# Zhang-Xin-Duke/multimodal-detection-consistency

Hardware: AMD Instinct MI355X
Metric: defended queries/sec (higher is better)
Workload: dtype bf16; 1 GPU; ViT-L/14 bf16, batch=512/GPU, N=8 variants, 1000000-row bf16 bank, encode + exact top-5 bank search + consistency (BASELINE configs[2]); global_batch=512, parallelism=dp1, text_packing=eot-packed + variant prefix sharing (bit-identical, see DESIGN.md), bank=gaussian + planted neighbours of the text rows

## Files before the change

multimodal-detection-consistency_amd/csrc/elementwise.hip:

```cpp
#include "common.hpp"
#include "kernels.hpp"
#include "launch.hpp"
#include "rows.hpp"

#ifndef TVC_LN_NT
#define TVC_LN_NT 7
#endif

template <bool F16>
__global__ __launch_bounds__(256) void layernorm_kernel(float* __restrict__ x, int64_t x_row_stride,
                                                        const int32_t* __restrict__ row_idx,
                                                        const uint16_t* __restrict__ delta,
                                                        const uint16_t* __restrict__ delta2, int write_x,
                                                        const float* __restrict__ g,
                                                        const float* __restrict__ b,
                                                        uint16_t* __restrict__ y, int rows, int d,
                                                        int delta_compact, float* __restrict__ xsum_out,
                                                        float* __restrict__ y32) {
    const int lane = row_lane();
    const int row = wave_row();
    if (row >= rows) return;
    const int64_t src_row = row_idx ? (int64_t)row_idx[row] : (int64_t)row;
    f32x4_t* xr = (f32x4_t*)(x + src_row * x_row_stride);
    const int64_t doff = delta_compact ? (int64_t)row * d : src_row * x_row_stride;
    const u32x2_t* dr = delta ? (const u32x2_t*)(delta + doff) : nullptr;
    const u32x2_t* dr2 = delta2 ? (const u32x2_t*)(delta2 + doff) : nullptr;
    const int nv = d >> 2;
    f32x4_t v[4] = {};
    float s = 0.f;
    for_pieces(lane, nv, [&](int i, int c) {
#if TVC_LN_NT & 1
        v[i] = __builtin_nontemporal_load(xr + c);
#else
        v[i] = xr[c];
#endif
        if (dr) {
#if TVC_LN_NT & 4
            v[i] += unpack4<F16>(__builtin_nontemporal_load(dr + c));
#else
            v[i] += unpack4<F16>(dr[c]);
#endif
        }
        if (dr2) v[i] += unpack4<F16>(dr2[c]);
#if TVC_LN_NT & 2
        if (write_x && (dr || dr2)) __builtin_nontemporal_store(v[i], xr + c);
#else
        if (write_x && (dr || dr2)) xr[c] = v[i];
#endif
        if (xsum_out) ((f32x4_t*)(xsum_out + (int64_t)row * d))[c] = v[i];
        s += piece_sum(v[i]);
    });
    const float mean = row_mean(s, d);
    const float rstd = row_rstd(v, mean, lane, nv, d);
    u32x2_t* yr = (u32x2_t*)(y + (int64_t)row * d);
    for_pieces(lane, nv, [&](int i, int c) {
        const f32x4_t o = ln_affine(v[i], mean, rstd, g, b, c);
        if (y32) ((f32x4_t*)(y32 + (int64_t)row * d))[c] = o;
        if (y) {
#if TVC_LN_NT & 8
            __builtin_nontemporal_store(pack4<F16>(o), yr + c);
#else
            yr[c] = pack4<F16>(o);
#endif
        }
    });
}

hipError_t launch_layernorm(float* x, int64_t x_row_stride, const int32_t* row_idx, const uint16_t* delta,
                            int write_x, const float* g, const float* b, uint16_t* y, int rows, int d,
                            hipStream_t stream, const uint16_t* delta2, int delta_compact, float* xsum_out, float* y32,
                            int f16) {
    if (d % 4 != 0 || d > 1024 || rows < 0) return hipErrorInvalidValue;
    if (rows == 0) return hipSuccess;
    return dispatch<true, false>(f16 != 0, [&](auto h) {
        return launch<layernorm_kernel<h.value>>(row_grid(rows), dim3(256), 0, stream, x, x_row_stride, row_idx, delta, delta2, write_x, g, b,
                                                 y, rows, d, delta_compact, xsum_out, y32);
    });
}

template <bool F16>
__global__ __launch_bounds__(256) void im2col_kernel(const float* __restrict__ pix,
                                                     uint16_t* __restrict__ out, int B, int S,
                                                     int patch, int Kp) {
    const int g = S / patch;
    const int P = g * g;
    const int chunks = Kp >> 3;
    const int64_t total = (int64_t)B * P * chunks;
    const int K = 3 * patch * patch;
    for (int64_t t = (int64_t)blockIdx.x * blockDim.x + threadIdx.x; t < total;
         t += (int64_t)gridDim.x * blockDim.x) {
        const int ch = (int)(t % chunks);
        const int64_t row = t / chunks;
        const int p = (int)(row % P);
        const int bimg = (int)(row / P);
        const int py = p / g, px = p - py * g;
        uint32_t w[4];
#pragma unroll
        for (int e = 0; e < 4; ++e) {
            float f[2];
#pragma unroll
            for (int h = 0; h < 2; ++h) {
                const int col = ch * 8 + e * 2 + h;
                float val = 0.f;
                if (col < K) {
                    const int c = col / (patch * patch);
                    const int rem = col - c * patch * patch;
                    const int ky = rem / patch, kx = rem - ky * patch;
                    val = pix[(((int64_t)bimg * 3 + c) * S + (py * patch + ky)) * S + (px * patch + kx)];
                }
                f[h] = val;
            }
            w[e] = Op16<F16>::pack2(f[0], f[1]);
        }
        *(u32x4_t*)(out + row * Kp + ch * 8) = u32x4_t{w[0], w[1], w[2], w[3]};
    }
}

template <bool F16>
__global__ __launch_bounds__(256) void im2col_rows_kernel(const float* __restrict__ pix, uint16_t* __restrict__ out,
                                                          int S, int patch, int Kp) {
    extern __shared__ __attribute__((aligned(16))) char im_smem[];
    uint16_t* tile = (uint16_t*)im_smem;
    const int g = S / patch;
    const int bimg = blockIdx.x / g, py = blockIdx.x - bimg * g;
    const int K = 3 * patch * patch;
    for (int i = threadIdx.x; i < g * (Kp - K); i += 256) {
        const int px = i / (Kp - K), c = K + (i - px * (Kp - K));
        tile[px * Kp + c] = 0;
    }
    const int s4 = S >> 2;
    const int total = 3 * patch * s4;
    for (int i = threadIdx.x; i < total; i += 256) {
        const int rowi = i / s4, x4 = i - rowi * s4;
        const int c = rowi / patch, ky = rowi - c * patch;
        const f32x4_t v = __builtin_nontemporal_load(
            (const f32x4_t*)(pix + (((int64_t)bimg * 3 + c) * S + (py * patch + ky)) * S) + x4);
#pragma unroll
        for (int e = 0; e < 4; ++e) {
            const int x = x4 * 4 + e;
            const int px = x / patch, kx = x - px * patch;
            tile[px * Kp + c * patch * patch + ky * patch + kx] = Op16<F16>::from_f32(v[e]);
        }
    }
    __syncthreads();
    const int chunks = (g * Kp) >> 3;
    u32x4_t* dst = (u32x4_t*)(out + ((int64_t)bimg * g * g + (int64_t)py * g) * Kp);
    for (int i = threadIdx.x; i < chunks; i += 256) dst[i] = ((const u32x4_t*)tile)[i];
}

hipError_t launch_im2col(const float* pix, uint16_t* out, int B, int image, int patch, int Kp,
                         hipStream_t stream, int f16) {
    if (B <= 0) return hipSuccess;
    const int g = image / patch;
    const size_t lds = (size_t)g * Kp * 2;
    if (image % 4 == 0 && Kp % 8 == 0 && lds <= 64 * 1024)
        return dispatch<true, false>(f16 != 0, [&](auto h) {
            return launch<im2col_rows_kernel<h.value>>(dim3(B * g), dim3(256), lds, stream, pix, out, image, patch, Kp);
        });
    const int64_t total = (int64_t)B * g * g * (Kp >> 3);
    return dispatch<true, false>(f16 != 0, [&](auto h) {
        return launch<im2col_kernel<h.value>>(stride_grid(total, 8192), dim3(256), 0, stream, pix, out, B, image, patch, Kp);
    });
}

__global__ __launch_bounds__(256) void assemble_lnpre_kernel(const float* __restrict__ patch_out,
                                                             const float* __restrict__ cls,
                                                             const float* __restrict__ pos,
                                                             const float* __restrict__ g,
                                                             const float* __restrict__ b,
                                                             float* __restrict__ x, int B, int T, int d) {
    const int lane = row_lane();
    const int64_t row = wave_row<int64_t>();
    if (row >= (int64_t)B * T) return;
    const int t = (int)(row % T);
    const int64_t bimg = row / T;
    const f32x4_t* src = (t == 0) ? (const f32x4_t*)cls
                                  : (const f32x4_t*)(patch_out + (bimg * (T - 1) + (t - 1)) * d);
    const f32x4_t* pr = (const f32x4_t*)(pos + (int64_t)t * d);
    const int nv = d >> 2;
    f32x4_t v[4] = {};
    float s = 0.f;
    for_pieces(lane, nv, [&](int i, int c) {
        v[i] = src[c] + pr[c];
        s += piece_sum(v[i]);
    });
    const float mean = row_mean(s, d);
    const float rstd = row_rstd(v, mean, lane, nv, d);
    f32x4_t* xr = (f32x4_t*)(x + row * d);
    for_pieces(lane, nv, [&](int i, int c) { xr[c] = ln_affine(v[i], mean, rstd, g, b, c); });
}

hipError_t launch_assemble_lnpre(const float* patch_out, const float* cls, const float* pos,
                                 const float* g, const float* b, float* x, int B, int T, int d,
                                 hipStream_t stream) {
    if (d % 4 != 0 || d > 1024) return hipErrorInvalidValue;
    const int64_t rows = (int64_t)B * T;
    if (rows == 0) return hipSuccess;
    return launch<assemble_lnpre_kernel>(row_grid(rows), dim3(256), 0, stream, patch_out, cls, pos, g, b, x, B, T, d);
}

__device__ __forceinline__ int first_max_pos(const int32_t* __restrict__ tok, int ctx, int lane) {
    int best = -1, best_t = 0;
    for (int tt = lane; tt < ctx; tt += 64) {
        const int v = tok[tt];
        if (v > best) { best = v; best_t = tt; }
    }
#pragma unroll
    for (int o = 32; o > 0; o >>= 1) {
        const int ov = __shfl_xor(best, o, 64);
        const int ot = __shfl_xor(best_t, o, 64);
        if (ov > best || (ov == best && ot < best_t)) { best = ov; best_t = ot; }
    }
    return best_t;
}

__global__ __launch_bounds__(256) void text_lens_kernel(const int32_t* __restrict__ tok, int32_t* __restrict__ starts,
                                                        int32_t* __restrict__ pfx, int32_t* __restrict__ lens,
                                                        int n_text, int ctx, int G) {
    const int lane = row_lane();
    const int n = wave_row();
    if (n >= n_text) return;
    int len = first_max_pos(tok + (int64_t)n * ctx, ctx, lane) + 1, p = 0;
    if (pfx) {
        const int bn = n / G * G;
        if (bn != n) {
            int bb = -1, bt = 0, mis = 0x7fffffff;
            for (int tt = lane; tt < ctx; tt += 64) {
                const int vb = tok[(int64_t)bn * ctx + tt], vn = tok[(int64_t)n * ctx + tt];
                if (vb > bb) { bb = vb; bt = tt; }
                if (vb != vn && tt < mis) mis = tt;
            }
#pragma unroll
            for (int o = 32; o > 0; o >>= 1) {
                const int ov = __shfl_xor(bb, o, 64);
                const int ot = __shfl_xor(bt, o, 64);
                if (ov > bb || (ov == bb && ot < bt)) { bb = ov; bt = ot; }
                const int om = __shfl_xor(mis, o, 64);
                mis = om < mis ? om : mis;
            }
            p = mis;
            if (p > len) p = len;
            if (p > bt + 1) p = bt + 1;
        }
        if (lane == 0) pfx[n] = p;
    }
    if (lane == 0) { starts[n] = len - p; lens[n] = len; }
}

__global__ __launch_bounds__(1024) void text_scan_kernel(int32_t* __restrict__ starts, int32_t* __restrict__ pfx,
                                                         const int32_t* __restrict__ lens, int n_text, int G) {
    __shared__ int part[1024];
// ... 192 lines not shown
```

multimodal-detection-consistency_amd/csrc/kernels.hpp:

```cpp
#pragma once
#include <hip/hip_runtime.h>
#include <stdint.h>
#include "host_plan.hpp"

enum { TVC_EPI_F32 = 0, TVC_EPI_BF16 = 1, TVC_EPI_GELU_BF16 = 2, TVC_EPI_RESID_F32 = 3 };

struct GemmLaunch {
    const uint16_t* A = nullptr;
    const uint16_t* B = nullptr;
    int64_t lda = 0, ldb = 0;
    int I = 0, J = 0, K = 0;
    int planes = 1;
    int a_plane_off[9] = {0, 0, 0, 0, 0, 0, 0, 0, 0};
    int b_plane_off[9] = {0, 0, 0, 0, 0, 0, 0, 0, 0};
    bool splitk_small = false;
    int splitk_fixed = 0;
    bool a_rows_padded = false;
    const float* bias = nullptr;
    void* out = nullptr;
    int64_t ldo = 0;
    int epilogue = TVC_EPI_F32;
    bool b_rows_padded = false;
    float* splitk_ws = nullptr;
    size_t splitk_ws_bytes = 0;
    bool f16 = false;
};
hipError_t launch_gemm_bf16(const GemmLaunch& L, hipStream_t stream);
inline GemmLaunch gemm_launch(const uint16_t* A, int64_t lda, int I, const uint16_t* B, int64_t ldb, int J, int K,
                              const float* bias, void* out, int64_t ldo, int epilogue) {
    GemmLaunch g;
    g.A = A; g.lda = lda; g.I = I; g.B = B; g.ldb = ldb; g.J = J; g.K = K;
    g.bias = bias; g.out = out; g.ldo = ldo; g.epilogue = epilogue;
    return g;
}
inline GemmLaunch gemm_launch_planes(const uint16_t* A, int64_t lda, int I, int bank_planes, const uint16_t* B, int J, int D,
                                     float* out, int64_t ldo) {
    GemmLaunch g = gemm_launch(A, lda, I, B, 2 * (int64_t)D, J, D, nullptr, out, ldo, TVC_EPI_F32);
    g.planes = bank_planes == 2 ? 3 : 2;
    g.b_plane_off[1] = D;
    g.a_plane_off[2] = D;
    return g;
}
inline GemmFormArgs form_args(const GemmLaunch& L) {
    GemmFormArgs a;
    a.I = L.I; a.J = L.J; a.K = L.K; a.planes = L.planes; a.lda = L.lda; a.ldb = L.ldb; a.epilogue = L.epilogue;
    a.splitk_small = L.splitk_small; a.splitk_fixed = L.splitk_fixed; a.has_ws = L.splitk_ws != nullptr;
    a.ws_bytes = L.splitk_ws_bytes; a.a_rows_padded = L.a_rows_padded; a.b_rows_padded = L.b_rows_padded;
    return a;
}

hipError_t launch_layernorm(float* x, int64_t x_row_stride, const int32_t* row_idx, const uint16_t* delta,
                            int write_x, const float* g, const float* b, uint16_t* y, int rows, int d,
                            hipStream_t stream, const uint16_t* delta2 = nullptr, int delta_compact = 0,
                            float* xsum_out = nullptr,
                            float* y32 = nullptr,
                            int f16 = 0);
hipError_t launch_im2col(const float* pix, uint16_t* out, int B, int image, int patch, int Kp,
                         hipStream_t stream, int f16 = 0);
hipError_t launch_assemble_lnpre(const float* patch_out, const float* cls, const float* pos,
                                 const float* g, const float* b, float* x, int B, int T, int d,
                                 hipStream_t stream);
hipError_t launch_text_embed(const int32_t* tok, const float* tok_emb, const float* pos, float* x,
                             int32_t* eot_row, const int32_t* starts, int n_text, int ctx, int d, int vocab,
                             hipStream_t stream, const int32_t* pfx = nullptr);
hipError_t launch_text_lens_scan(const int32_t* tok, int32_t* starts, int32_t* pfx, int n_text, int ctx, int G,
                                 hipStream_t stream, int32_t* lens_ws);
hipError_t launch_l2norm_rows(float* x, int rows, int d, hipStream_t stream);
hipError_t launch_gelu_erf_16(uint16_t* x, int64_t n, int f16, hipStream_t stream);
hipError_t launch_gelu_erf_f32(float* x, int64_t n, hipStream_t stream);
hipError_t launch_split_planes(const float* x, uint16_t* out, int64_t rows, int d, int planes,
                               hipStream_t stream);
hipError_t launch_gather_rows(const uint16_t* bank, int64_t ld, int planes, int D, int64_t R,
                              const int32_t* idx, int64_t idx_offset, int n, float* out,
                              hipStream_t stream);

hipError_t launch_attention(const uint16_t* qkv, uint16_t* out, const int32_t* starts, int n_seq,
                            int seq_len, int heads, int causal, hipStream_t stream, const int32_t* pfx = nullptr,
                            int pool_mode = 0, const int32_t* pool_row = nullptr,
                            int f16 = 0);

struct BankSearchLaunch {
    const uint16_t* bank = nullptr;
    int64_t ldb = 0;
    int64_t R = 0;
    int D = 0;
    int bank_planes = 1;
    const uint16_t* qplanes = nullptr;
    const float* rows = nullptr;
    const float* bank_bounds = nullptr;
    bool allow_filter = true;
    bool q_rows_padded = false;
    int M = 0;
    int k = 0;
    float count_thr = 0.f;
    int64_t idx_offset = 0;
    float* s0 = nullptr;
    float* gmax = nullptr;
    float* tau = nullptr;
    void* cand = nullptr;
    int32_t* cand_cnt = nullptr;
    float* mom_part = nullptr;
    int32_t* overflow = nullptr;
    int n_sample = 0, sample_stride = 1, S = 0, cap = 0;
    int32_t* topk_idx = nullptr;
    float* topk_sim = nullptr;
    float* moments = nullptr;
};
hipError_t launch_bank_search(const BankSearchLaunch& L, hipStream_t stream);
hipError_t launch_bank_bounds(const uint16_t* bank, int64_t ld, int planes, int D, int64_t R, float* bounds,
                              hipStream_t stream);
hipError_t launch_bank_search_dense(const BankSearchLaunch& L, float* sims_ws, int block_rows, hipStream_t stream);
hipError_t launch_topk_merge(const int32_t* idx_parts, const float* sim_parts, const float* feat_parts,
                             const float* mom_parts, int W, int M, int k, int kf, int D,
                             int32_t* idx_out, float* sim_out, float* feat_out, float* mom_out,
                             hipStream_t stream);

struct ConsistencyParams {
    int reference_count;
    float similarity_threshold;
    int retrieval_top_k;
    float dup_threshold;
    float w_text_variants, w_consistency;
    float w_exp[4];
};
// ... 63 lines not shown
```

multimodal-detection-consistency_amd/csrc/rows.hpp:

```cpp
#pragma once
#include "common.hpp"

#define ROWS_PER_BLOCK 4
#define LN_EPS 1e-5f

__device__ __forceinline__ int row_lane() { return threadIdx.x & 63; }
template <class R = int>
__device__ __forceinline__ R wave_row() { return (R)blockIdx.x * ROWS_PER_BLOCK + (threadIdx.x >> 6); }

template <class F>
__device__ __forceinline__ void for_pieces(int lane, int nv, F&& f) {
#pragma unroll
    for (int i = 0; i < 4; ++i) {
        const int c = lane + 64 * i;
        if (c < nv) f(i, c);
    }
}

__device__ __forceinline__ float piece_sum(const f32x4_t v) { return (v[0] + v[1]) + (v[2] + v[3]); }
__device__ __forceinline__ float row_mean(float s, int d) { return wave_sum(s) / (float)d; }
template <bool EXACT = false>
__device__ __forceinline__ float row_rstd(const f32x4_t (&v)[4], float mean, int lane, int nv, int d) {
    float q = 0.f;
    for_pieces(lane, nv, [&](int i, int) {
#pragma unroll
        for (int t = 0; t < 4; ++t) {
#pragma clang fp contract(off)
            const float dl = v[i][t] - mean;
            q += dl * dl;
        }
    });
    const float var = wave_sum(q) / (float)d + LN_EPS;
    return EXACT ? 1.0f / sqrtf(var) : rsqrtf(var);
}

__device__ __forceinline__ f32x4_t ln_affine(const f32x4_t v, float mean, float rstd, const float* __restrict__ g,
                                             const float* __restrict__ b, int c) {
    const f32x4_t gg = ((const f32x4_t*)g)[c];
    const f32x4_t bb = ((const f32x4_t*)b)[c];
    f32x4_t o;
#pragma unroll
    for (int t = 0; t < 4; ++t) o[t] = fmaf((v[t] - mean) * rstd, gg[t], bb[t]);
    return o;
}

template <class Store>
__device__ __forceinline__ void ln_bwd_tail(f32x4_t (&v)[4], const f32x4_t (&g)[4], float mean, float rstd, int lane, int nv,
                                            int d, Store&& store) {
    float sg = 0.f, sgx = 0.f;
    for_pieces(lane, nv, [&](int i, int) {
#pragma unroll
        for (int t = 0; t < 4; ++t) {
            v[i][t] = (v[i][t] - mean) * rstd;
            sg += g[i][t];
            sgx = fmaf(g[i][t], v[i][t], sgx);
        }
    });
    const float c1 = wave_sum(sg) / (float)d, c2 = wave_sum(sgx) / (float)d;
    for_pieces(lane, nv, [&](int i, int c) {
        f32x4_t o;
#pragma unroll
        for (int t = 0; t < 4; ++t) o[t] = rstd * (g[i][t] - c1 - v[i][t] * c2);
        store(c, o);
    });
}

__device__ __forceinline__ float gelu_erf(float x) { return 0.5f * x * (1.0f + erff(x * 0.70710678118654752f)); }
__device__ __forceinline__ float quick_gelu_sigmoid(float x) {
    return __builtin_amdgcn_rcpf(1.0f + __builtin_amdgcn_exp2f(-2.4554670f * x));
}
__device__ __forceinline__ float quick_gelu(float x) { return x * quick_gelu_sigmoid(x); }
__device__ __forceinline__ float quick_gelu_grad(float x) {
    const float s = quick_gelu_sigmoid(x);
    return s + 1.702f * x * s * (1.0f - s);
}
__device__ __forceinline__ float quick_gelu_exact(float x) { return x / (1.0f + expf(-1.702f * x)); }

template <bool F16 = false>
__device__ __forceinline__ f32x4_t unpack4(const u32x2_t w) {
    return f32x4_t{Op16<F16>::lo(w[0]), Op16<F16>::hi(w[0]), Op16<F16>::lo(w[1]), Op16<F16>::hi(w[1])};
}
template <bool F16 = false>
__device__ __forceinline__ u32x2_t pack4(const f32x4_t f) {
    return u32x2_t{Op16<F16>::pack2(f[0], f[1]), Op16<F16>::pack2(f[2], f[3])};
}
template <bool F16 = false>
__device__ __forceinline__ void unpack8(const u32x4_t v, float* f) {
#pragma unroll
    for (int i = 0; i < 4; ++i) {
        f[2 * i] = Op16<F16>::lo(v[i]);
        f[2 * i + 1] = Op16<F16>::hi(v[i]);
    }
}
template <bool F16 = false>
__device__ __forceinline__ u32x4_t pack8(const float* f) {
    return u32x4_t{Op16<F16>::pack2(f[0], f[1]), Op16<F16>::pack2(f[2], f[3]), Op16<F16>::pack2(f[4], f[5]),
// ... 3 lines not shown
```

multimodal-detection-consistency_amd/csrc/tvc_abi.cpp:

```cpp
#include "handle.hpp"

#include <cstdlib>

namespace {

bool tower_ok(const tvc_tower_arch& a) {
    return a.width > 0 && a.layers > 0 && a.heads > 0 && a.width == a.heads * 64 && a.width % 64 == 0 &&
           a.width <= 1024 && a.mlp > 0 && a.mlp % 64 == 0 && (a.act == TVC_ACT_QUICK_GELU || a.act == TVC_ACT_GELU);
}

struct PoolBufs { uint16_t *Hc, *D1c, *H2c, *MLPc, *D2c; };
PoolBufs pool_bufs(tvc_handle* h, const tvc_tower_arch& a, int n_seq, int wso) {
    uint16_t* p = (uint16_t*)h->ws[WS_POOL + wso].p;
    const size_t nd = ((size_t)n_seq + 256) * a.width;
    PoolBufs b;
    b.Hc = p; b.D1c = p + nd; b.H2c = p + 2 * nd; b.D2c = p + 3 * nd; b.MLPc = p + 4 * nd;
    return b;
}
size_t pool_bytes(const tvc_tower_arch& a, int n_seq) {
    return (((size_t)n_seq + 256) * a.width * 4 + ((size_t)n_seq + 256) * a.mlp) * 2;
}

struct GradSave {
    float* x;
    uint16_t* qkv;
    uint16_t* d1;
    uint16_t* u;
};

int run_layers(tvc_handle* h, const tvc_tower_arch& a, const tvc_layer_weights* lw, int n_seq, int seq_len,
               int causal, const int32_t* starts, int total_rows, int wso, hipStream_t st,
               const int32_t* pfx = nullptr, int pool_mode = 0, const int32_t* pool_row = nullptr,
               int64_t pool_x_stride = 0, const GradSave* gs = nullptr, bool f16 = false) {
    const int d = a.width;
    const int rows = starts ? total_rows : n_seq * seq_len;
    float* X = (float*)h->ws[WS_X + wso].p;
    uint16_t* H = (uint16_t*)h->ws[WS_H + wso].p;
    uint16_t* QKV = (uint16_t*)h->ws[WS_QKV + wso].p;
    uint16_t* MLP = (uint16_t*)h->ws[WS_MLP + wso].p;
    uint16_t* D1 = (uint16_t*)h->ws[WS_DELTA + wso].p;
    uint16_t* D2 = (uint16_t*)h->ws[WS_DELTA2 + wso].p;
    bool pending = false;
    for (int l = 0; l < a.layers; ++l) {
        const tvc_layer_weights& w = lw[l];
        {
            ProfScope ps(h, st, TVC_PROF_ROWOPS, (double)rows * d * (pending ? 14.0 : 6.0));
            HIP_TRY(launch_layernorm(X, d, nullptr, pending ? D1 : nullptr, 1, w.ln1_g, w.ln1_b, H, rows, d, st,
                                     pending ? D2 : nullptr, 0, gs ? gs->x + (size_t)l * rows * d : nullptr, nullptr, f16));
        }
        if (gs) {
            QKV = gs->qkv + (size_t)l * rows * 3 * d;
            D1 = gs->d1 + (size_t)l * rows * d;
        }
        GemmLaunch g = gemm_launch(w.wqkv, d, 3 * d, H, d, rows, d, w.bqkv, QKV, 3 * d, TVC_EPI_BF16);
        g.b_rows_padded = true; g.f16 = f16;
        g.splitk_small = gs != nullptr;
        HIP_TRY(timed_gemm(h, g, st, WS_SPLITK + wso));
        if (pool_mode && l == a.layers - 1) {
            const PoolBufs pb = pool_bufs(h, a, n_seq, wso);
            {
                const double avg_len = starts ? (double)rows / n_seq : (double)seq_len;
                ProfScope ps(h, st, TVC_PROF_ATTENTION, 4.0 * n_seq * a.heads * avg_len * 64);
                HIP_TRY(launch_attention(QKV, pb.Hc, starts, n_seq, seq_len, a.heads, causal, st, pfx, pool_mode, pool_row, f16));
            }
            g = gemm_launch(w.wo, d, d, pb.Hc, d, n_seq, d, w.bo, pb.D1c, d, TVC_EPI_BF16);
            g.b_rows_padded = true; g.f16 = f16;
            HIP_TRY(timed_gemm(h, g, st, WS_SPLITK + wso));
            HIP_TRY(launch_layernorm(X, pool_row ? d : pool_x_stride, pool_row, pb.D1c, 0, w.ln2_g, w.ln2_b, pb.H2c, n_seq, d,
                                     st, nullptr, 1, nullptr, nullptr, f16));
            g = gemm_launch(w.w1, d, a.mlp, pb.H2c, d, n_seq, d, w.b1, pb.MLPc, a.mlp,
                            a.act == TVC_ACT_GELU ? TVC_EPI_BF16 : TVC_EPI_GELU_BF16);
            g.b_rows_padded = true; g.f16 = f16;
            HIP_TRY(timed_gemm(h, g, st, WS_SPLITK + wso));
            if (a.act == TVC_ACT_GELU)
                HIP_TRY(launch_gelu_erf_16(pb.MLPc, (int64_t)n_seq * a.mlp, f16, st));
            g = gemm_launch(w.w2, a.mlp, d, pb.MLPc, a.mlp, n_seq, a.mlp, w.b2, pb.D2c, d, TVC_EPI_BF16);
            g.b_rows_padded = true; g.f16 = f16;
            HIP_TRY(timed_gemm(h, g, st, WS_SPLITK + wso));
            return TVC_OK;
        }
        {
            const double avg_len = starts ? (double)rows / n_seq : (double)seq_len;
            const double fl = 4.0 * n_seq * a.heads * avg_len * avg_len * 64 * (causal ? 0.5 : 1.0);
            ProfScope ps(h, st, TVC_PROF_ATTENTION, fl);
            HIP_TRY(launch_attention(QKV, H, starts, n_seq, seq_len, a.heads, causal, st, pfx, 0, nullptr, f16));
        }
        g = gemm_launch(w.wo, d, d, H, d, rows, d, w.bo, D1, d, TVC_EPI_BF16);
        g.b_rows_padded = true; g.f16 = f16; g.splitk_small = gs != nullptr;
        HIP_TRY(timed_gemm(h, g, st, WS_SPLITK + wso));
        {
            ProfScope ps(h, st, TVC_PROF_ROWOPS, (double)rows * d * 8.0);
            HIP_TRY(launch_layernorm(X, d, nullptr, D1, 0, w.ln2_g, w.ln2_b, H, rows, d, st, nullptr, 0, nullptr, nullptr, f16));
        }
        uint16_t* U = gs ? gs->u + (size_t)l * rows * a.mlp : MLP;
        g = gemm_launch(w.w1, d, a.mlp, H, d, rows, d, w.b1, U, a.mlp, gs || a.act == TVC_ACT_GELU ? TVC_EPI_BF16 : TVC_EPI_GELU_BF16);
        g.b_rows_padded = true; g.f16 = f16; g.splitk_small = gs != nullptr;
        HIP_TRY(timed_gemm(h, g, st, WS_SPLITK + wso));
        if (gs) {
            HIP_TRY(launch_gelu_fwd(U, MLP, (int64_t)rows * a.mlp, st));
        } else if (a.act == TVC_ACT_GELU) {
            ProfScope ps(h, st, TVC_PROF_ROWOPS, (double)rows * a.mlp * 4.0);
            HIP_TRY(launch_gelu_erf_16(MLP, (int64_t)rows * a.mlp, f16, st));
        }
        g = gemm_launch(w.w2, a.mlp, d, MLP, a.mlp, rows, a.mlp, w.b2, D2, d, TVC_EPI_BF16);
        g.b_rows_padded = true; g.f16 = f16; g.splitk_small = gs != nullptr;
        HIP_TRY(timed_gemm(h, g, st, WS_SPLITK + wso));
        pending = true;
    }
    return TVC_OK;
}

int ensure_tower_ws(tvc_handle* h, const tvc_tower_arch& a, int64_t rows, int n_seq, int wso) {
// ... 6 lines not shown
    if ((rc = ensure(h, (Slot)(WS_CLS + wso), (size_t)n_seq * a.width * 2))) return rc;
    if ((rc = ensure(h, (Slot)(WS_DELTA + wso), (size_t)rows * a.width * 2))) return rc;
    if ((rc = ensure(h, (Slot)(WS_DELTA2 + wso), (size_t)rows * a.width * 2))) return rc;
    if ((rc = ensure(h, (Slot)(WS_SPLITK + wso), (size_t)256 * 256 * 256 * 4))) return rc;
    if ((rc = ensure(h, (Slot)(WS_POOL + wso), pool_bytes(a, n_seq)))) return rc;
    return TVC_OK;
}

int patch_stem(tvc_handle* h, const char* fn, const float* pix, int n, bool f16, const float** patch_out, hipStream_t st) {
    const tvc_model_desc& m = h->desc;
    const int gside = m.image_size / m.patch, P = gside * gside, d = m.vision.width;
    const int Kp = (3 * m.patch * m.patch + 63) / 64 * 64;
    uint16_t* Pm = (uint16_t*)h->ws[WS_PATCH].p;
    float* po = (float*)h->ws[WS_MLP].p;
    if ((size_t)n * P * d * 4 > h->ws[WS_MLP].n) return fail(h, TVC_E_INVALID, std::string(fn) + ": mlp < 2*width unsupported");
    HIP_TRY(launch_im2col(pix, Pm, n, m.image_size, m.patch, Kp, st, f16));
    GemmLaunch g = gemm_launch((f16 ? h->vision16 : h->vision).w.patch_w, Kp, d, Pm, Kp, n * P, Kp, nullptr, po, d, TVC_EPI_F32);
    g.b_rows_padded = true; g.f16 = f16;
    HIP_TRY(timed_gemm(h, g, st, WS_SPLITK));
    *patch_out = po;
    return TVC_OK;
}


int tower_begin(tvc_handle* h, bool text, const char* fn, int n_seq, float** X) {
    const int mode = h->tower_precision;
    auto missing = [&](const char* tail) {
        return fail(h, TVC_E_STATE, std::string(mode == 3 ? fn : text ? "tvc_encode_text" : "tvc_encode_image") +
                                        ": TVC_OPT_TOWER_PRECISION = " + std::to_string(mode) + " needs tvc_set_weights_f" +
                                        (mode == 3 ? "16" : "32") + (text ? " (text)" : " (vision)") + tail);
    };
    const bool has32 = text ? h->text32.set : h->vision32.set;
    if (mode == 1) return has32 ? precise_ensure(h, text, n_seq, X) : missing("");
    if (mode == 2) {
        if (!has32 || !h->split_ready || (text ? h->tsplit : h->vsplit).empty()) return missing(" before the option is set");
        return split_ensure(h, text, n_seq, X);
    }
    if (mode == 3 && !(text ? h->text16.set : h->vision16.set)) return missing("");
    const tvc_model_desc& m = h->desc;
    const int gside = m.image_size / m.patch, P = gside * gside, T = P + 1;
    const int Kp = (3 * m.patch * m.patch + 63) / 64 * 64;
    int rc;
    if (text) {
        if ((rc = ensure_tower_ws(h, m.text, (int64_t)n_seq * m.ctx, n_seq, WS_TOWER_N))) return rc;
    } else {
        if ((rc = ensure_tower_ws(h, m.vision, (int64_t)n_seq * T, n_seq, 0))) return rc;
        if ((rc = ensure(h, WS_PATCH, ((size_t)n_seq * P + 512) * Kp * 2))) return rc;
    }
    *X = (float*)h->ws[WS_X + (text ? WS_TOWER_N : 0)].p;
    return TVC_OK;
}

int tower_layers(tvc_handle* h, bool text, int n_seq, int seq_len, const int32_t* starts, int total_rows, const int32_t* pfx,
                 bool pool, int64_t x_stride, const int32_t* row_idx, hipStream_t st) {
    if (h->tower_precision == 1) return precise_layers(h, text, n_seq, seq_len, st);
    if (h->tower_precision == 2) return split_layers(h, text, n_seq, seq_len, starts, total_rows, pfx, st);
    const bool f16 = h->tower_precision == 3;
    const tvc_layer_weights* lw = text ? (f16 ? h->text16 : h->text).w.layers : (f16 ? h->vision16 : h->vision).w.layers;
    return run_layers(h, text ? h->desc.text : h->desc.vision, lw, n_seq, seq_len, text ? 1 : 0, starts, total_rows,
                      text ? WS_TOWER_N : 0, st, pfx, pool ? (text ? 2 : 1) : 0, row_idx, x_stride, nullptr, f16);
}

int tower_head(tvc_handle* h, bool text, int64_t x_stride, const int32_t* row_idx, int rows, bool pool, float* out, bool hidden,
               hipStream_t st) {
    if (h->tower_precision == 1) return precise_head(h, text, x_stride, row_idx, rows, out, hidden, st);
    if (h->tower_precision == 2) return split_head(h, text, x_stride, row_idx, rows, out, hidden, st);
    const bool f16 = h->tower_precision == 3;
    const tvc_model_desc& m = h->desc;
    const tvc_tower_arch& a = text ? m.text : m.vision;
    const int d = a.width, wso = text ? WS_TOWER_N : 0;
    const tvc_vision_weights& vw = (f16 ? h->vision16 : h->vision).w;
    const tvc_text_weights& tw = (f16 ? h->text16 : h->text).w;
    const PoolBufs pb = pool ? pool_bufs(h, a, rows, wso) : PoolBufs{};
    uint16_t* Hc = hidden ? nullptr : (uint16_t*)h->ws[WS_CLS + wso].p;
    HIP_TRY(launch_layernorm((float*)h->ws[WS_X + wso].p, x_stride, row_idx, pool ? pb.D1c : (const uint16_t*)h->ws[WS_DELTA + wso].p,
                             0, text ? tw.ln_final_g : vw.ln_post_g, text ? tw.ln_final_b : vw.ln_post_b, Hc, rows, d, st,
                             pool ? pb.D2c : (const uint16_t*)h->ws[WS_DELTA2 + wso].p, pool ? 1 : 0, nullptr,
                             hidden ? out : nullptr, f16));
    if (hidden) return TVC_OK;
    GemmLaunch g = gemm_launch(text ? tw.proj : vw.proj, d, m.embed_dim, Hc, d, rows, d, nullptr, out, m.embed_dim, TVC_EPI_F32);
    g.f16 = f16;
    HIP_TRY(timed_gemm(h, g, st, WS_SPLITK + wso));
    return TVC_OK;
}

int encode_text(tvc_handle* h, const char* fn, const int32_t* tok_dev, int32_t Tn, float* out_dev, int32_t normalize, bool hidden,
                void* stream) {
    if (!h) return TVC_E_INVALID;
    if (!h->text.set) return fail(h, TVC_E_STATE, std::string(fn) + ": handle has no text tower");
    if (Tn < 0 || (Tn > 0 && (!tok_dev || !out_dev))) return fail(h, TVC_E_INVALID, std::string(fn) + ": bad arguments");
    hipStream_t st = (hipStream_t)stream;
    const tvc_model_desc& m = h->desc;
    const int d = m.text.width, ctx = m.ctx;
    if (Tn == 0) return TVC_OK;
    int chunk = Tn < h->max_chunk_texts ? Tn : h->max_chunk_texts;
    const int mode = h->tower_precision;
    const bool pack = h->pack_text && !hidden && mode != 1;
    const bool pool = h->pooled_last && !hidden && (mode == 0 || mode == 3);
    const int G = (pack && h->text_group >= 2 && Tn % h->text_group == 0) ? h->text_group : 0;
    if (G && chunk >= G) chunk = chunk / G * G;
    const bool share = G && chunk % G == 0;
    float* X;
    int rc;
    if ((rc = tower_begin(h, true, fn, chunk, &X))) return rc;
    if (share && (rc = ensure(h, WS_PFX, (size_t)chunk * 2 * 4))) return rc;
    if ((rc = ensure(h, WS_EOT, (size_t)chunk * 4))) return rc;
    if (pack && (rc = ensure(h, WS_STARTS, (size_t)(chunk + 2) * 4))) return rc;
    if (pack && (rc = ensure(h, WS_LENS, (size_t)chunk * 4))) return rc;
    int32_t* eot = (int32_t*)h->ws[WS_EOT].p;
    for (int t0 = 0; t0 < Tn; t0 += chunk) {
        const int n = (Tn - t0 < chunk) ? Tn - t0 : chunk;
        const int32_t* tok = tok_dev + (size_t)t0 * ctx;
        const int32_t* starts = nullptr;
// ... 63 lines not shown
        const tvc_model_desc& d = *desc;
        if (!tower_ok(d.text) || d.ctx <= 0 || d.ctx > 288 || d.vocab <= 0 || d.embed_dim % 64 != 0 || !text->layers) {
            delete nh;
            return fail(h, TVC_E_INVALID, "tvc_create: unsupported text geometry");
        }
        nh->text.assign(*text, d.text.layers);
    }
    *out = nh;
    return TVC_OK;
}

void tvc_destroy(tvc_handle* h) {
    if (!h) return;
    tvc_sd_free(h);
    tvc_split_free(h);
    for (auto& b : h->ws) if (b.p) (void)hipFree(b.p);
    for (void* p : h->wT) if (p) (void)hipFree(p);
    for (auto& bk : h->banks) {
        if (bk.owned) (void)hipFree(bk.owned);
        if (bk.bounds) (void)hipFree(bk.bounds);
    }
    delete h;
}

uint64_t tvc_workspace_bytes(tvc_handle* h) {
    if (!h) return 0;
    uint64_t n = 0;
    for (auto& b : h->ws) n += b.n;
    return n;
}

int tvc_encode_image(tvc_handle* h, const float* pix_dev, int32_t B, float* out_dev, int32_t normalize,
                     void* stream) {
    if (!h) return TVC_E_INVALID;
    if (!h->vision.set) return fail(h, TVC_E_STATE, "tvc_encode_image: handle has no vision tower");
    if (B < 0 || (B > 0 && (!pix_dev || !out_dev))) return fail(h, TVC_E_INVALID, "tvc_encode_image: bad arguments");
    hipStream_t st = (hipStream_t)stream;
    const tvc_model_desc& m = h->desc;
    const int gside = m.image_size / m.patch, T = gside * gside + 1, d = m.vision.width;
    const int chunk = B < h->max_chunk_images ? B : h->max_chunk_images;
    if (B == 0) return TVC_OK;
    const int mode = h->tower_precision;
    const bool pool = h->pooled_last && (mode == 0 || mode == 3);
    float* X;
    int rc;
    if ((rc = tower_begin(h, false, "tvc_encode_image", chunk, &X))) return rc;
    for (int b0 = 0; b0 < B; b0 += chunk) {
        const int n = (B - b0 < chunk) ? B - b0 : chunk;
        const float* pix = pix_dev + (size_t)b0 * 3 * m.image_size * m.image_size;
        const float* patch_out;
        rc = mode == 1 ? precise_stem(h, pix, n, &patch_out, st) : mode == 2 ? split_stem(h, pix, n, &patch_out, st)
                       : patch_stem(h, "tvc_encode_image", pix, n, mode == 3, &patch_out, st);
        if (rc) return rc;
        auto assemble = [&](const auto& w) {
            return launch_assemble_lnpre(patch_out, w.cls, w.pos, w.ln_pre_g, w.ln_pre_b, X, n, T, d, st);
        };
        HIP_TRY(mode == 1 || mode == 2 ? assemble(h->vision32.w) : assemble((mode == 3 ? h->vision16 : h->vision).w));
        if ((rc = tower_layers(h, false, n, T, nullptr, 0, nullptr, pool, (int64_t)T * d, nullptr, st))) return rc;
        float* out = out_dev + (size_t)b0 * m.embed_dim;
        if ((rc = tower_head(h, false, (int64_t)T * d, nullptr, n, pool, out, false, st))) return rc;
        if (normalize) HIP_TRY(launch_l2norm_rows(out, n, m.embed_dim, st));
    }
    return TVC_OK;
}

int tvc_encode_text(tvc_handle* h, const int32_t* tok_dev, int32_t Tn, float* out_dev, int32_t normalize,
                    void* stream) {
    return encode_text(h, "tvc_encode_text", tok_dev, Tn, out_dev, normalize, false, stream);
}

int tvc_encode_text_hidden(tvc_handle* h, const int32_t* tok_dev, int32_t Tn, float* out_dev, void* stream) {
    return encode_text(h, "tvc_encode_text_hidden", tok_dev, Tn, out_dev, 0, true, stream);
}

int tvc_bank_set(tvc_handle* h, const void* bank_dev, int64_t R, int32_t D, int32_t dtype, void* stream) {
    if (!h) return TVC_E_INVALID;
    BankSlot& bk = h->banks[h->cur_bank];
    if (R < 0 || R > 0x7fffffffLL || D <= 0 || D % 64 != 0 || (R > 0 && !bank_dev))
        return fail(h, TVC_E_INVALID, "tvc_bank_set: need 0 <= R < 2^31 and D % 64 == 0");
    if (bk.owned) { HIP_TRY(hipFree(bk.owned)); bk.owned = nullptr; }
    bk.bank = nullptr; bk.R = 0; bk.D = D;
    if (dtype == TVC_DTYPE_BF16) {
        bk.bank = (const uint16_t*)bank_dev; bk.planes = 1;
    } else if (dtype == TVC_DTYPE_F32) {
        if (R > 0) {
            HIP_TRY(hipMalloc(&bk.owned, (size_t)R * 2 * D * 2));
            HIP_TRY(launch_split_planes((const float*)bank_dev, (uint16_t*)bk.owned, R, D, 2, (hipStream_t)stream));
        }
        bk.bank = (const uint16_t*)bk.owned; bk.planes = 2;
    } else {
        return fail(h, TVC_E_INVALID, "tvc_bank_set: dtype must be TVC_DTYPE_BF16 or TVC_DTYPE_F32");
    }
    if (!bk.bounds) HIP_TRY(hipMalloc((void**)&bk.bounds, 8));
    HIP_TRY(launch_bank_bounds(bk.bank, (int64_t)bk.planes * D, bk.planes, D, R, bk.bounds,
                               (hipStream_t)stream));
    bk.R = R;
    return TVC_OK;
}

int tvc_bank_select(tvc_handle* h, int32_t slot) {
    if (!h) return TVC_E_INVALID;
    if (slot < 0 || slot >= TVC_MAX_BANKS) return fail(h, TVC_E_INVALID, "tvc_bank_select: slot must be in [0, TVC_MAX_BANKS)");
    h->cur_bank = slot;
    return TVC_OK;
}

int tvc_bank_search(tvc_handle* h, const float* rows_dev, int32_t M, int32_t k, float count_thr,
                    int64_t idx_offset, int32_t* topk_idx_dev, float* topk_sim_dev, float* moments_dev,
                    void* stream) {
    if (!h) return TVC_E_INVALID;
    BankSlot& bk = h->banks[h->cur_bank];
// ... 167 lines not shown
    if (!h->wT.empty()) return TVC_OK;
    const tvc_model_desc& m = h->desc;
    const tvc_tower_arch& a = m.vision;
    const int d = a.width, Kp = (3 * m.patch * m.patch + 63) / 64 * 64;
    auto tr = [&](const uint16_t* w, int R, int C, void** out) -> int {
        HIP_TRY(hipMalloc(out, (size_t)R * C * 2));
        HIP_TRY(launch_transpose_bf16(w, (uint16_t*)*out, R, C, st));
        return TVC_OK;
    };
    std::vector<void*> t((size_t)a.layers * 4 + 2, nullptr);
    int rc = TVC_OK;
    for (int l = 0; l < a.layers && !rc; ++l) {
        const tvc_layer_weights& w = h->vision.w.layers[l];
        if ((rc = tr(w.wqkv, 3 * d, d, &t[l * 4 + 0]))) break;
        if ((rc = tr(w.wo, d, d, &t[l * 4 + 1]))) break;
        if ((rc = tr(w.w1, a.mlp, d, &t[l * 4 + 2]))) break;
        if ((rc = tr(w.w2, d, a.mlp, &t[l * 4 + 3]))) break;
    }
    if (!rc) rc = tr(h->vision.w.proj, m.embed_dim, d, &t[(size_t)a.layers * 4]);
    if (!rc) rc = tr(h->vision.w.patch_w, d, Kp, &t[(size_t)a.layers * 4 + 1]);
    if (rc) { for (void* p : t) if (p) (void)hipFree(p); return rc; }
    h->wT = t;
    return TVC_OK;
}
}

int tvc_encode_image_grad(tvc_handle* h, const float* pix_dev, int32_t B, float* out_dev, int32_t normalize, void* stream) {
    if (!h) return TVC_E_INVALID;
    if (!h->vision.set) return fail(h, TVC_E_STATE, "tvc_encode_image_grad: handle has no vision tower");
    if (B < 1 || !pix_dev || !out_dev) return fail(h, TVC_E_INVALID, "tvc_encode_image_grad: bad arguments");
    if (B > h->max_chunk_images) return fail(h, TVC_E_INVALID, "tvc_encode_image_grad: B exceeds TVC_OPT_MAX_CHUNK_IMAGES (one pass only)");
    if (h->desc.vision.act != TVC_ACT_QUICK_GELU) return fail(h, TVC_E_INVALID, "tvc_encode_image_grad: only QuickGELU towers have a backward pass");
    hipStream_t st = (hipStream_t)stream;
    const tvc_model_desc& m = h->desc;
    const tvc_tower_arch& a = m.vision;
    const int gside = m.image_size / m.patch, P = gside * gside, T = P + 1, d = a.width;
    const int Kp = (3 * m.patch * m.patch + 63) / 64 * 64;
    const int64_t rows = (int64_t)B * T;
    int rc;
    if ((rc = ensure_tower_ws(h, a, rows, B, 0))) return rc;
    if ((rc = ensure(h, WS_PATCH, ((size_t)B * P + 512) * Kp * 2))) return rc;
    const size_t per_layer = (size_t)rows * ((size_t)d * 4 + (size_t)3 * d * 2 + (size_t)d * 2 + (size_t)a.mlp * 2);
    if ((rc = ensure(h, WS_GSAVE, (size_t)a.layers * per_layer + 256))) return rc;
    GradSave gs;
    gs.x = (float*)h->ws[WS_GSAVE].p;
    gs.qkv = (uint16_t*)(gs.x + (size_t)a.layers * rows * d);
    gs.d1 = gs.qkv + (size_t)a.layers * rows * 3 * d;
    gs.u = gs.d1 + (size_t)a.layers * rows * d;
    if ((rc = ensure(h, WS_GOUT, (size_t)B * m.embed_dim * 4))) return rc;
    if ((rc = ensure(h, WS_GXL, (size_t)B * d * 4))) return rc;
    const float* patch_out;
    if ((rc = patch_stem(h, "tvc_encode_image_grad", pix_dev, B, false, &patch_out, st))) return rc;
    const tvc_vision_weights& vw = h->vision.w;
    HIP_TRY(launch_assemble_lnpre(patch_out, vw.cls, vw.pos, vw.ln_pre_g, vw.ln_pre_b, (float*)h->ws[WS_X].p, B, T, d, st));
    if ((rc = run_layers(h, a, vw.layers, B, T, 0, nullptr, 0, 0, st, nullptr, 0, nullptr, 0, &gs))) return rc;
    uint16_t* Hc = (uint16_t*)h->ws[WS_CLS].p;
    HIP_TRY(launch_layernorm((float*)h->ws[WS_X].p, (int64_t)T * d, nullptr, gs.d1 + (size_t)(a.layers - 1) * rows * d, 0,
                             vw.ln_post_g, vw.ln_post_b, Hc, B, d, st, (const uint16_t*)h->ws[WS_DELTA2].p, 0,
                             (float*)h->ws[WS_GXL].p));
    HIP_TRY(timed_gemm(h, gemm_launch(vw.proj, d, m.embed_dim, Hc, d, B, d, nullptr, h->ws[WS_GOUT].p, m.embed_dim, TVC_EPI_F32), st,
                       WS_SPLITK));
    HIP_TRY(hipMemcpyAsync(out_dev, h->ws[WS_GOUT].p, (size_t)B * m.embed_dim * 4, hipMemcpyDeviceToDevice, st));
    if (normalize) HIP_TRY(launch_l2norm_rows(out_dev, B, m.embed_dim, st));
    h->grad_B = B; h->grad_normalize = normalize; h->grad_pix = pix_dev;
    return TVC_OK;
}

int tvc_encode_image_backward(tvc_handle* h, const float* grad_out_dev, float* grad_pix_dev, void* stream) {
    if (!h) return TVC_E_INVALID;
    if (!h->vision.set || h->grad_B < 1) return fail(h, TVC_E_STATE, "tvc_encode_image_backward: call tvc_encode_image_grad first");
    if (!grad_out_dev || !grad_pix_dev) return fail(h, TVC_E_INVALID, "tvc_encode_image_backward: NULL buffer");
    hipStream_t st = (hipStream_t)stream;
    const tvc_model_desc& m = h->desc;
    const tvc_tower_arch& a = m.vision;
    const int B = h->grad_B, gside = m.image_size / m.patch, P = gside * gside, T = P + 1, d = a.width, D = m.embed_dim;
    const int Kp = (3 * m.patch * m.patch + 63) / 64 * 64;
    const int64_t rows = (int64_t)B * T;
    const int64_t rows_pad = (rows + 255) / 256 * 256 + 256;
    int rc;
    if ((rc = build_transposed_weights(h, st))) return rc;
    if ((rc = ensure(h, WS_GDX, (size_t)rows_pad * d * 4))) return rc;
    if ((rc = ensure(h, WS_G16, (size_t)rows_pad * d * 2))) return rc;
    if ((rc = ensure(h, WS_GMLP2, (size_t)rows_pad * a.mlp * 2))) return rc;
    if ((rc = ensure(h, WS_GDQKV, (size_t)rows_pad * 3 * d * 2))) return rc;
    if ((rc = ensure(h, WS_GSTATS, (size_t)rows * a.heads * 16))) return rc;
    if ((rc = ensure(h, WS_GSMALL, ((size_t)B + 256) * (D + d) * 2))) return rc;
    if ((rc = ensure(h, WS_GPATCH, ((size_t)B * P + 512) * (size_t)(Kp > d ? Kp : d) * 4))) return rc;
    uint16_t* H = (uint16_t*)h->ws[WS_H].p;
    uint16_t* D2 = (uint16_t*)h->ws[WS_DELTA2].p;
    float* dX = (float*)h->ws[WS_GDX].p;
    uint16_t* G16 = (uint16_t*)h->ws[WS_G16].p;
    uint16_t* dM = (uint16_t*)h->ws[WS_GMLP2].p;
    uint16_t* dQKV = (uint16_t*)h->ws[WS_GDQKV].p;
    auto gemm = [&](const void* A, int64_t lda, int I, const uint16_t* Bm, int64_t ldb, int J, int K, void* out, int64_t ldo,
                    int epi) -> int {
        GemmLaunch g = gemm_launch((const uint16_t*)A, lda, I, Bm, ldb, J, K, nullptr, out, ldo, epi);
        g.b_rows_padded = true;
        g.splitk_small = true;
        HIP_TRY(timed_gemm(h, g, st, WS_SPLITK));
        return TVC_OK;
    };
    uint16_t* dP16 = (uint16_t*)h->ws[WS_GSMALL].p;
    uint16_t* dHc = dP16 + ((size_t)B + 256) * D;
    HIP_TRY(launch_l2norm_bwd((const float*)h->ws[WS_GOUT].p, grad_out_dev, dP16, B, D, h->grad_normalize, st));
    if ((rc = gemm(h->wT[(size_t)a.layers * 4], D, d, dP16, D, B, D, dHc, d, TVC_EPI_BF16))) return rc;
    HIP_TRY(hipMemsetAsync(dX, 0, (size_t)rows * d * 4, st));
    HIP_TRY(hipMemsetAsync(G16, 0, (size_t)rows * d * 2, st));
    HIP_TRY(launch_layernorm_bwd((const float*)h->ws[WS_GXL].p, d, nullptr, dHc, 0, h->vision.w.ln_post_g, nullptr, dX, G16, B, d,
// ... 252 lines not shown
```

Baseline: 5246 queries/s.

## Fuse vision stem assembly into first layernorm and skip unneeded Q projection rows

Folds the CLS/pos-embedding assembly plus ln_pre into the first layer's ln1 kernel, so X is written once and never re-read before ln1. In the pooled final layer, the QKV GEMM skips the Q columns for all rows. Q is then computed only for the pooled rows, either by gathering them into a compact buffer, running a small GEMM and scattering the result back, or through a strided GEMM. This cuts memory traffic and final-layer GEMM work, at the cost of extra small launches and more code-path complexity.

```diff
diff --git a/multimodal-detection-consistency_amd/csrc/elementwise.hip b/multimodal-detection-consistency_amd/csrc/elementwise.hip
--- a/multimodal-detection-consistency_amd/csrc/elementwise.hip
+++ b/multimodal-detection-consistency_amd/csrc/elementwise.hip
@@ -7,7 +7,7 @@
 #define TVC_LN_NT 7
 #endif
 
-template <bool F16>
+template <bool F16, bool STEM = false>
 __global__ __launch_bounds__(256) void layernorm_kernel(float* __restrict__ x, int64_t x_row_stride,
                                                         const int32_t* __restrict__ row_idx,
                                                         const uint16_t* __restrict__ delta,
@@ -16,11 +16,11 @@
                                                         const float* __restrict__ b,
                                                         uint16_t* __restrict__ y, int rows, int d,
                                                         int delta_compact, float* __restrict__ xsum_out,
-                                                        float* __restrict__ y32) {
+                                                        float* __restrict__ y32, StemRows stem) {
     const int lane = row_lane();
     const int row = wave_row();
     if (row >= rows) return;
-    const int64_t src_row = row_idx ? (int64_t)row_idx[row] : (int64_t)row;
+    const int64_t src_row = (!STEM && row_idx) ? (int64_t)row_idx[row] : (int64_t)row;
     f32x4_t* xr = (f32x4_t*)(x + src_row * x_row_stride);
     const int64_t doff = delta_compact ? (int64_t)row * d : src_row * x_row_stride;
     const u32x2_t* dr = delta ? (const u32x2_t*)(delta + doff) : nullptr;
@@ -28,7 +28,18 @@
     const int nv = d >> 2;
     f32x4_t v[4] = {};
     float s = 0.f;
-    for_pieces(lane, nv, [&](int i, int c) {
+    if (STEM) {
+        stem_row(stem, row, lane, nv, d, v);
+        for_pieces(lane, nv, [&](int i, int c) {
+#if TVC_LN_NT & 2
+            __builtin_nontemporal_store(v[i], xr + c);
+#else
+            xr[c] = v[i];
+#endif
+            if (xsum_out) ((f32x4_t*)(xsum_out + (int64_t)row * d))[c] = v[i];
+            s += piece_sum(v[i]);
+        });
+    } else for_pieces(lane, nv, [&](int i, int c) {
 #if TVC_LN_NT & 1
         v[i] = __builtin_nontemporal_load(xr + c);
 #else
@@ -74,7 +85,17 @@
     if (rows == 0) return hipSuccess;
     return dispatch<true, false>(f16 != 0, [&](auto h) {
         return launch<layernorm_kernel<h.value>>(row_grid(rows), dim3(256), 0, stream, x, x_row_stride, row_idx, delta, delta2, write_x, g, b,
-                                                 y, rows, d, delta_compact, xsum_out, y32);
+                                                 y, rows, d, delta_compact, xsum_out, y32, StemRows{});
+    });
+}
+
+hipError_t launch_layernorm_stem(const StemRows& stem, float* x, const float* g, const float* b, uint16_t* y, int rows, int d,
+                                 hipStream_t stream, float* xsum_out, int f16) {
+    if (d % 4 != 0 || d > 1024 || rows < 0 || stem.T < 1 || rows % stem.T != 0) return hipErrorInvalidValue;
+    if (rows == 0) return hipSuccess;
+    return dispatch<true, false>(f16 != 0, [&](auto h) {
+        return launch<layernorm_kernel<h.value, true>>(row_grid(rows), dim3(256), 0, stream, x, (int64_t)d, nullptr, nullptr, nullptr, 0, g, b,
+                                                       y, rows, d, 0, xsum_out, nullptr, stem);
     });
 }
 
@@ -172,22 +193,11 @@
     const int lane = row_lane();
     const int64_t row = wave_row<int64_t>();
     if (row >= (int64_t)B * T) return;
-    const int t = (int)(row % T);
-    const int64_t bimg = row / T;
-    const f32x4_t* src = (t == 0) ? (const f32x4_t*)cls
-                                  : (const f32x4_t*)(patch_out + (bimg * (T - 1) + (t - 1)) * d);
-    const f32x4_t* pr = (const f32x4_t*)(pos + (int64_t)t * d);
     const int nv = d >> 2;
     f32x4_t v[4] = {};
-    float s = 0.f;
-    for_pieces(lane, nv, [&](int i, int c) {
-        v[i] = src[c] + pr[c];
-        s += piece_sum(v[i]);
-    });
-    const float mean = row_mean(s, d);
-    const float rstd = row_rstd(v, mean, lane, nv, d);
+    stem_row(StemRows{patch_out, cls, pos, g, b, T}, row, lane, nv, d, v);
     f32x4_t* xr = (f32x4_t*)(x + row * d);
-    for_pieces(lane, nv, [&](int i, int c) { xr[c] = ln_affine(v[i], mean, rstd, g, b, c); });
+    for_pieces(lane, nv, [&](int i, int c) { xr[c] = v[i]; });
 }
 
 hipError_t launch_assemble_lnpre(const float* patch_out, const float* cls, const float* pos,
@@ -197,6 +207,24 @@
     const int64_t rows = (int64_t)B * T;
     if (rows == 0) return hipSuccess;
     return launch<assemble_lnpre_kernel>(row_grid(rows), dim3(256), 0, stream, patch_out, cls, pos, g, b, x, B, T, d);
+}
+
+__global__ __launch_bounds__(256) void copy_rows16_kernel(const uint16_t* __restrict__ src, int64_t src_stride,
+                                                          const int32_t* __restrict__ src_idx, uint16_t* __restrict__ dst,
+                                                          int64_t dst_stride, const int32_t* __restrict__ dst_idx, int n, int d) {
+    const int lane = row_lane();
+    const int row = wave_row();
+    if (row >= n) return;
+    const u32x4_t* s = (const u32x4_t*)(src + (src_idx ? (int64_t)src_idx[row] : (int64_t)row) * src_stride);
+    u32x4_t* o = (u32x4_t*)(dst + (dst_idx ? (int64_t)dst_idx[row] : (int64_t)row) * dst_stride);
+    for (int c = lane; c < (d >> 3); c += 64) o[c] = s[c];
+}
+
+hipError_t launch_copy_rows16(const uint16_t* src, int64_t src_stride, const int32_t* src_idx, uint16_t* dst, int64_t dst_stride,
+                              const int32_t* dst_idx, int n, int d, hipStream_t stream) {
+    if (d % 8 != 0 || src_stride % 8 != 0 || dst_stride % 8 != 0 || n < 0) return hipErrorInvalidValue;
+    if (n == 0) return hipSuccess;
+    return launch<copy_rows16_kernel>(row_grid(n), dim3(256), 0, stream, src, src_stride, src_idx, dst, dst_stride, dst_idx, n, d);
 }
 
 __device__ __forceinline__ int first_max_pos(const int32_t* __restrict__ tok, int ctx, int lane) {
diff --git a/multimodal-detection-consistency_amd/csrc/kernels.hpp b/multimodal-detection-consistency_amd/csrc/kernels.hpp
--- a/multimodal-detection-consistency_amd/csrc/kernels.hpp
+++ b/multimodal-detection-consistency_amd/csrc/kernels.hpp
@@ -55,6 +55,14 @@
                             float* xsum_out = nullptr,
                             float* y32 = nullptr,
                             int f16 = 0);
+struct StemRows {
+    const float* patch_out;
+    const float *cls, *pos;
+    const float *g, *b;
+    int T;
+};
+hipError_t launch_layernorm_stem(const StemRows& stem, float* x, const float* g, const float* b, uint16_t* y, int rows, int d,
+                                 hipStream_t stream, float* xsum_out = nullptr, int f16 = 0);
 hipError_t launch_im2col(const float* pix, uint16_t* out, int B, int image, int patch, int Kp,
                          hipStream_t stream, int f16 = 0);
 hipError_t launch_assemble_lnpre(const float* patch_out, const float* cls, const float* pos,
@@ -70,6 +78,8 @@
 hipError_t launch_gelu_erf_f32(float* x, int64_t n, hipStream_t stream);
 hipError_t launch_split_planes(const float* x, uint16_t* out, int64_t rows, int d, int planes,
                                hipStream_t stream);
+hipError_t launch_copy_rows16(const uint16_t* src, int64_t src_stride, const int32_t* src_idx, uint16_t* dst, int64_t dst_stride,
+                              const int32_t* dst_idx, int n, int d, hipStream_t stream);
 hipError_t launch_gather_rows(const uint16_t* bank, int64_t ld, int planes, int D, int64_t R,
                               const int32_t* idx, int64_t idx_offset, int n, float* out,
                               hipStream_t stream);
diff --git a/multimodal-detection-consistency_amd/csrc/rows.hpp b/multimodal-detection-consistency_amd/csrc/rows.hpp
--- a/multimodal-detection-consistency_amd/csrc/rows.hpp
+++ b/multimodal-detection-consistency_amd/csrc/rows.hpp
@@ -1,5 +1,6 @@
 #pragma once
 #include "common.hpp"
+#include "kernels.hpp"
 
 #define ROWS_PER_BLOCK 4
 #define LN_EPS 1e-5f
@@ -42,6 +43,21 @@
 #pragma unroll
     for (int t = 0; t < 4; ++t) o[t] = fmaf((v[t] - mean) * rstd, gg[t], bb[t]);
     return o;
+}
+
+__device__ __forceinline__ void stem_row(const StemRows& s, int64_t row, int lane, int nv, int d, f32x4_t (&v)[4]) {
+    const int t = (int)(row % s.T);
+    const int64_t bimg = row / s.T;
+    const f32x4_t* src = (t == 0) ? (const f32x4_t*)s.cls : (const f32x4_t*)(s.patch_out + (bimg * (s.T - 1) + (t - 1)) * d);
+    const f32x4_t* pr = (const f32x4_t*)(s.pos + (int64_t)t * d);
+    float sum = 0.f;
+    for_pieces(lane, nv, [&](int i, int c) {
+        v[i] = src[c] + pr[c];
+        sum += piece_sum(v[i]);
+    });
+    const float mean = row_mean(sum, d);
+    const float rstd = row_rstd(v, mean, lane, nv, d);
+    for_pieces(lane, nv, [&](int i, int c) { v[i] = ln_affine(v[i], mean, rstd, s.g, s.b, c); });
 }
 
 template <class Store>
diff --git a/multimodal-detection-consistency_amd/csrc/tvc_abi.cpp b/multimodal-detection-consistency_amd/csrc/tvc_abi.cpp
--- a/multimodal-detection-consistency_amd/csrc/tvc_abi.cpp
+++ b/multimodal-detection-consistency_amd/csrc/tvc_abi.cpp
@@ -31,7 +31,7 @@
 int run_layers(tvc_handle* h, const tvc_tower_arch& a, const tvc_layer_weights* lw, int n_seq, int seq_len,
                int causal, const int32_t* starts, int total_rows, int wso, hipStream_t st,
                const int32_t* pfx = nullptr, int pool_mode = 0, const int32_t* pool_row = nullptr,
-               int64_t pool_x_stride = 0, const GradSave* gs = nullptr, bool f16 = false) {
+               int64_t pool_x_stride = 0, const GradSave* gs = nullptr, bool f16 = false, const StemRows* stem = nullptr) {
     const int d = a.width;
     const int rows = starts ? total_rows : n_seq * seq_len;
     float* X = (float*)h->ws[WS_X + wso].p;
@@ -45,19 +45,36 @@
         const tvc_layer_weights& w = lw[l];
         {
             ProfScope ps(h, st, TVC_PROF_ROWOPS, (double)rows * d * (pending ? 14.0 : 6.0));
-            HIP_TRY(launch_layernorm(X, d, nullptr, pending ? D1 : nullptr, 1, w.ln1_g, w.ln1_b, H, rows, d, st,
-                                     pending ? D2 : nullptr, 0, gs ? gs->x + (size_t)l * rows * d : nullptr, nullptr, f16));
+            if (l == 0 && stem)
+                HIP_TRY(launch_layernorm_stem(*stem, X, w.ln1_g, w.ln1_b, H, rows, d, st, gs ? gs->x : nullptr, f16));
+            else
+                HIP_TRY(launch_layernorm(X, d, nullptr, pending ? D1 : nullptr, 1, w.ln1_g, w.ln1_b, H, rows, d, st,
+                                         pending ? D2 : nullptr, 0, gs ? gs->x + (size_t)l * rows * d : nullptr, nullptr, f16));
         }
         if (gs) {
             QKV = gs->qkv + (size_t)l * rows * 3 * d;
             D1 = gs->d1 + (size_t)l * rows * d;
         }
-        GemmLaunch g = gemm_launch(w.wqkv, d, 3 * d, H, d, rows, d, w.bqkv, QKV, 3 * d, TVC_EPI_BF16);
+        const bool pooled_last = pool_mode && l == a.layers - 1;
+        const int q_skip = pooled_last ? d : 0;
+        GemmLaunch g = gemm_launch(w.wqkv + (size_t)q_skip * d, d, 3 * d - q_skip, H, d, rows, d, w.bqkv + q_skip, QKV + q_skip,
+                                   3 * d, TVC_EPI_BF16);
         g.b_rows_padded = true; g.f16 = f16;
         g.splitk_small = gs != nullptr;
         HIP_TRY(timed_gemm(h, g, st, WS_SPLITK + wso));
-        if (pool_mode && l == a.layers - 1) {
+        if (pooled_last) {
             const PoolBufs pb = pool_bufs(h, a, n_seq, wso);
+            if (pool_row) {
+                HIP_TRY(launch_copy_rows16(H, d, pool_row, pb.H2c, d, nullptr, n_seq, d, st));
+                g = gemm_launch(w.wqkv, d, d, pb.H2c, d, n_seq, d, w.bqkv, pb.D1c, d, TVC_EPI_BF16);
+                g.b_rows_padded = true; g.f16 = f16;
+                HIP_TRY(timed_gemm(h, g, st, WS_SPLITK + wso));
+                HIP_TRY(launch_copy_rows16(pb.D1c, d, nullptr, QKV, 3 * (int64_t)d, pool_row, n_seq, d, st));
+            } else {
+                g = gemm_launch(w.wqkv, d, d, H, pool_x_stride, n_seq, d, w.bqkv, QKV, 3 * pool_x_stride, TVC_EPI_BF16);
+                g.f16 = f16;
+                HIP_TRY(timed_gemm(h, g, st, WS_SPLITK + wso));
+            }
             {
                 const double avg_len = starts ? (double)rows / n_seq : (double)seq_len;
                 ProfScope ps(h, st, TVC_PROF_ATTENTION, 4.0 * n_seq * a.heads * avg_len * 64);
@@ -170,13 +187,13 @@
 }
 
 int tower_layers(tvc_handle* h, bool text, int n_seq, int seq_len, const int32_t* starts, int total_rows, const int32_t* pfx,
-                 bool pool, int64_t x_stride, const int32_t* row_idx, hipStream_t st) {
+                 bool pool, int64_t x_stride, const int32_t* row_idx, hipStream_t st, const StemRows* stem = nullptr) {
     if (h->tower_precision == 1) return precise_layers(h, text, n_seq, seq_len, st);
     if (h->tower_precision == 2) return split_layers(h, text, n_seq, seq_len, starts, total_rows, pfx, st);
     const bool f16 = h->tower_precision == 3;
     const tvc_layer_weights* lw = text ? (f16 ? h->text16 : h->text).w.layers : (f16 ? h->vision16 : h->vision).w.layers;
     return run_layers(h, text ? h->desc.text : h->desc.vision, lw, n_seq, seq_len, text ? 1 : 0, starts, total_rows,
-                      text ? WS_TOWER_N : 0, st, pfx, pool ? (text ? 2 : 1) : 0, row_idx, x_stride, nullptr, f16);
+                      text ? WS_TOWER_N : 0, st, pfx, pool ? (text ? 2 : 1) : 0, row_idx, x_stride, nullptr, f16, stem);
 }
 
 int tower_head(tvc_handle* h, bool text, int64_t x_stride, const int32_t* row_idx, int rows, bool pool, float* out, bool hidden,
@@ -346,11 +363,14 @@
         rc = mode == 1 ? precise_stem(h, pix, n, &patch_out, st) : mode == 2 ? split_stem(h, pix, n, &patch_out, st)
                        : patch_stem(h, "tvc_encode_image", pix, n, mode == 3, &patch_out, st);
         if (rc) return rc;
-        auto assemble = [&](const auto& w) {
-            return launch_assemble_lnpre(patch_out, w.cls, w.pos, w.ln_pre_g, w.ln_pre_b, X, n, T, d, st);
-        };
-        HIP_TRY(mode == 1 || mode == 2 ? assemble(h->vision32.w) : assemble((mode == 3 ? h->vision16 : h->vision).w));
-        if ((rc = tower_layers(h, false, n, T, nullptr, 0, nullptr, pool, (int64_t)T * d, nullptr, st))) return rc;
+        const tvc_vision_weights& vw = (mode == 3 ? h->vision16 : h->vision).w;
+        const StemRows stem{patch_out, vw.cls, vw.pos, vw.ln_pre_g, vw.ln_pre_b, T};
+        if (mode == 1 || mode == 2) {
+            const auto& w = h->vision32.w;
+            HIP_TRY(launch_assemble_lnpre(patch_out, w.cls, w.pos, w.ln_pre_g, w.ln_pre_b, X, n, T, d, st));
+        }
+        if ((rc = tower_layers(h, false, n, T, nullptr, 0, nullptr, pool, (int64_t)T * d, nullptr, st,
+                               mode == 1 || mode == 2 ? nullptr : &stem))) return rc;
         float* out = out_dev + (size_t)b0 * m.embed_dim;
         if ((rc = tower_head(h, false, (int64_t)T * d, nullptr, n, pool, out, false, st))) return rc;
         if (normalize) HIP_TRY(launch_l2norm_rows(out, n, m.embed_dim, st));
@@ -624,8 +644,8 @@
     const float* patch_out;
     if ((rc = patch_stem(h, "tvc_encode_image_grad", pix_dev, B, false, &patch_out, st))) return rc;
     const tvc_vision_weights& vw = h->vision.w;
-    HIP_TRY(launch_assemble_lnpre(patch_out, vw.cls, vw.pos, vw.ln_pre_g, vw.ln_pre_b, (float*)h->ws[WS_X].p, B, T, d, st));
-    if ((rc = run_layers(h, a, vw.layers, B, T, 0, nullptr, 0, 0, st, nullptr, 0, nullptr, 0, &gs))) return rc;
+    const StemRows stem{patch_out, vw.cls, vw.pos, vw.ln_pre_g, vw.ln_pre_b, T};
+    if ((rc = run_layers(h, a, vw.layers, B, T, 0, nullptr, 0, 0, st, nullptr, 0, nullptr, 0, &gs, false, &stem))) return rc;
     uint16_t* Hc = (uint16_t*)h->ws[WS_CLS].p;
     HIP_TRY(launch_layernorm((float*)h->ws[WS_X].p, (int64_t)T * d, nullptr, gs.d1 + (size_t)(a.layers - 1) * rows * d, 0,
                              vw.ln_post_g, vw.ln_post_b, Hc, B, d, st, (const uint16_t*)h->ws[WS_DELTA2].p, 0,
```

Result: no change. 5262 queries/s (median of 6 runs) (+0.3%).
